# xingyizhou/CenterNet

Measured on AMD Instinct MI355X. Metric: images/sec whole-node, 512x512 ctdet, higher is better.
Workload: dtype f32s; 1 GPU; ctdet resdcn_18 512x512, batch 32 per GPU (BASELINE configs[1]), network + fused sigmoid/peak-NMS/top-K decode, K=100; global_batch=32, parallelism=image-sharded x1

## Files before the change

### centernet_amd/csrc/cn_proj.hip

```cpp
#include "cn_internal.h"
#include "cn_tuning.h"

namespace {

constexpr int J_NT = 256;
constexpr int J_NB = 4;
constexpr int J_ROW = 144;
constexpr int J_STRIP = 32 * J_ROW;
constexpr int J_SLOT = 32 * 128;
static_assert(J_STRIP <= 2 * J_SLOT, "the epilogue strip aliases the input slots");

struct JArgs {
    const char *x;
    const char *w;
    int ncb;
    const float *scale, *shift;
    char *y;
    int M, Ho, Wo, H, W, stride;
    int in_pitchB, out_pitchB, cout_pad, nchunk, Cout, relu;
    uint32_t *range;
};

typedef _Float16 j_f16x8 __attribute__((ext_vector_type(8)));

typedef __attribute__((address_space(3))) void j_lds_void;
typedef __attribute__((address_space(1))) const void j_glb_void;

template <bool OUT_PLAIN, int J_PRE>
__global__ __launch_bounds__(J_NT, 2) void proj1x1_kernel(const JArgs a)
{
    constexpr int J_WAVE = J_PRE * J_SLOT;
    constexpr int J_SS = 4 * J_WAVE;
    extern __shared__ __attribute__((aligned(128))) char smem[];
    const int tid = threadIdx.x, lane = tid & 63;
    const int wave = __builtin_amdgcn_readfirstlane(tid >> 6);
    const int l31 = lane & 31, h = lane >> 5;
    const int n0 = (int)blockIdx.y * (32 * J_NB);
    {
        const int which = tid >> 7, c = tid & 127;
        const float *src = which ? a.shift : a.scale;
        float v = which ? 0.f : 1.f;
        if (src && n0 + c < a.Cout) v = src[n0 + c];
        reinterpret_cast<float *>(smem + J_SS)[tid] = v;
    }
    const int m_base = (int)blockIdx.x * 128 + wave * 32;
    unsigned src_off[4];
#pragma unroll
    for (int q = 0; q < 4; ++q) {
        const int p = 8 * q + (lane >> 3);
        const int mc = min(m_base + p, a.M - 1);
        const int ox = mc % a.Wo, t1 = mc / a.Wo, oy = t1 % a.Ho, b = t1 / a.Ho;
        const unsigned pin = (unsigned)((b * a.H + oy * a.stride) * a.W + ox * a.stride);
        src_off[q] = pin * (unsigned)a.in_pitchB + (unsigned)(((lane & 7) ^ ((p >> 1) & 7)) * 16);
    }
    char *wbase = smem + wave * J_WAVE;
    auto dma = [&](int slot, int c) {
#pragma unroll
        for (int q = 0; q < 4; ++q)
            __builtin_amdgcn_global_load_lds((j_glb_void *)(a.x + src_off[q] + (unsigned)c * 128u),
                                             (j_lds_void *)(wbase + slot * J_SLOT + q * 1024), 16, 0, 0);
    };
#pragma unroll
    for (int c = 0; c < J_PRE; ++c)
        if (c < a.nchunk) dma(c, c);
    const int sw = (l31 >> 1) & 7;
    const int rd = l31 * 128;
    const char *wl = a.w + (size_t)(n0 >> 5) * 4096 + (unsigned)lane * 16u;
    const size_t chunkB = (size_t)a.ncb * 4096;
    const int nbv = min(J_NB, a.ncb - (n0 >> 5));

    cn_f32x16 acc[J_NB];
#pragma unroll
    for (int nb = 0; nb < J_NB; ++nb)
#pragma unroll
        for (int r = 0; r < 16; ++r) acc[nb][r] = 0.f;
    __syncthreads();

    for (int c = 0; c < a.nchunk; ++c) {
        const int slot = c & (J_PRE - 1);
        j_f16x8 af[2][4];
        auto load_a = [&](int set, int nb) {
            const char *g = wl + (size_t)c * chunkB + (size_t)min(nb, nbv - 1) * 4096;
#pragma unroll
            for (int qd = 0; qd < 4; ++qd) af[set][qd] = *reinterpret_cast<const j_f16x8 *>(g + qd * 1024);
        };
        load_a(0, 0);
        {
            const int younger = min(a.nchunk - 1 - c, J_PRE - 1);
            if (J_PRE > 2 && younger >= 3) asm volatile("s_waitcnt vmcnt(16)" ::: "memory");
            else if (J_PRE > 2 && younger == 2) asm volatile("s_waitcnt vmcnt(12)" ::: "memory");
            else if (younger == 1) asm volatile("s_waitcnt vmcnt(8)" ::: "memory");
            else asm volatile("s_waitcnt vmcnt(4)" ::: "memory");
        }
        j_f16x8 bf[4];
        {
            const char *sp = wbase + slot * J_SLOT + rd;
            bf[0] = *reinterpret_cast<const j_f16x8 *>(sp + (((0 + h) ^ sw) << 4));
            bf[1] = *reinterpret_cast<const j_f16x8 *>(sp + (((2 + h) ^ sw) << 4));
            bf[2] = *reinterpret_cast<const j_f16x8 *>(sp + (((4 + h) ^ sw) << 4));
            bf[3] = *reinterpret_cast<const j_f16x8 *>(sp + (((6 + h) ^ sw) << 4));
        }
#pragma unroll
        for (int nb = 0; nb < J_NB; ++nb) {
            const int set = nb & 1;
            if (nb + 1 < J_NB) load_a(set ^ 1, nb + 1);
            __builtin_amdgcn_sched_barrier(0);
#pragma unroll
            for (int kh = 0; kh < 2; ++kh) {
                acc[nb] = __builtin_amdgcn_mfma_f32_32x32x16_f16(af[set][2 + kh], bf[kh], acc[nb], 0, 0, 0);
                acc[nb] = __builtin_amdgcn_mfma_f32_32x32x16_f16(af[set][kh], bf[2 + kh], acc[nb], 0, 0, 0);
                acc[nb] = __builtin_amdgcn_mfma_f32_32x32x16_f16(af[set][kh], bf[kh], acc[nb], 0, 0, 0);
            }
            __builtin_amdgcn_sched_barrier(0);
        }
        if (c + J_PRE < a.nchunk) {
            asm volatile("s_waitcnt lgkmcnt(0)" ::: "memory");
            dma(slot, c + J_PRE);
        }
    }
    asm volatile("s_waitcnt vmcnt(0) lgkmcnt(0)" ::: "memory");

    char *strip = smem + wave * J_WAVE;
    const float *ss = reinterpret_cast<const float *>(smem + J_SS);
    float rng_out = 0.f;
    const int rrow = lane >> 3, rcol = lane & 7;
    const float floor_v = a.relu ? 0.f : -__builtin_inff();
#pragma unroll
    for (int nb = 0; nb < J_NB; ++nb) {
        if (n0 + 32 * nb >= a.cout_pad) break;
#pragma unroll
        for (int g = 0; g < 4; ++g) {
            const cn_f32x4 sc = *reinterpret_cast<const cn_f32x4 *>(ss + 32 * nb + 8 * g + 4 * h);
            const cn_f32x4 sh = *reinterpret_cast<const cn_f32x4 *>(ss + 128 + 32 * nb + 8 * g + 4 * h);
            cn_f32x4 v;
#pragma unroll
            for (int e = 0; e < 4; ++e) v[e] = fmaxf(acc[nb][4 * g + e] * sc[e] + sh[e], floor_v);
            if (OUT_PLAIN) {
                *reinterpret_cast<cn_f32x4 *>(strip + l31 * J_ROW + (8 * g + 4 * h) * 4) = v;
            } else {
                cn_rng_upd4(rng_out, v);
                cn_f16x4v h4, l4;
                cn_split4(v, h4, l4);
                *reinterpret_cast<cn_f16x4v *>(strip + l31 * J_ROW + (8 * g + 4 * h) * 2) = h4;
                *reinterpret_cast<cn_f16x4v *>(strip + l31 * J_ROW + 64 + (8 * g + 4 * h) * 2) = l4;
            }
        }
        asm volatile("" ::: "memory");
#pragma unroll
        for (int k = 0; k < 4; ++k) {
            const int row = 8 * k + rrow;
            const cn_f32x4 v = *reinterpret_cast<const cn_f32x4 *>(strip + row * J_ROW + rcol * 16);
            const int mo = (int)blockIdx.x * 128 + wave * 32 + row;
            if (mo < a.M)
                *reinterpret_cast<cn_f32x4 *>(a.y + (size_t)mo * a.out_pitchB + (size_t)(n0 + 32 * nb) * 4 + rcol * 16) = v;
        }
        asm volatile("" ::: "memory");
    }
    if (!OUT_PLAIN) cn_rng_commit(a.range, 0, rng_out);
}

}

bool cn_proj1x1_takes(const ConvCall &c)
{
    if (!cn_knobs.proj) return false;
    if ((c.Cin & 31) || (c.in_pitch & 31) || (c.out_pitch & 31) || (c.stride != 1 && c.stride != 2)) return false;
    if (c.out_pitch < c.cout_pad) return false;
    if ((size_t)c.B * c.H * c.W * c.in_pitch * 4 >= ((size_t)1 << 32)) return false;
    return c.Cin <= 1024 && c.Cout >= 32;
}

int cn_proj1x1_f32s(const ConvCall &c, hipStream_t st)
{
    JArgs a = {};
    a.x = (const char *)c.x; a.w = (const char *)c.w + (size_t)c.cout_pad * c.Cin * 4; a.scale = c.scale; a.shift = c.shift;
    a.y = (char *)c.y;
    a.H = c.H; a.W = c.W; a.stride = c.stride;
    a.Ho = c.Ho; a.Wo = c.Wo;
    a.M = c.B * a.Ho * a.Wo;
    a.in_pitchB = c.in_pitch * 4; a.out_pitchB = c.out_pitch * 4;
    a.cout_pad = c.cout_pad;
    a.ncb = a.cout_pad / 32;
    a.nchunk = c.Cin / 32;
    a.Cout = c.Cout; a.relu = c.relu;
    a.range = c.ctl ? c.ctl->range : nullptr;
    const dim3 grid((unsigned)cn_cdiv(a.M, 128), (unsigned)cn_cdiv(a.cout_pad, 32 * J_NB));
    const int pre = a.nchunk <= 2 ? 2 : 4;
    const int lds = 4 * pre * J_SLOT + 2 * 128 * 4;
    if (c.out_plain && pre == 2) {
        CN_SET_MAX_LDS_ONCE((proj1x1_kernel<true, 2>), 4 * 2 * J_SLOT + 1024);
        hipLaunchKernelGGL((proj1x1_kernel<true, 2>), grid, dim3(J_NT), lds, st, a);
    } else if (c.out_plain) {
        CN_SET_MAX_LDS_ONCE((proj1x1_kernel<true, 4>), 4 * 4 * J_SLOT + 1024);
        hipLaunchKernelGGL((proj1x1_kernel<true, 4>), grid, dim3(J_NT), lds, st, a);
    } else if (pre == 2) {
        CN_SET_MAX_LDS_ONCE((proj1x1_kernel<false, 2>), 4 * 2 * J_SLOT + 1024);
        hipLaunchKernelGGL((proj1x1_kernel<false, 2>), grid, dim3(J_NT), lds, st, a);
    } else {
        CN_SET_MAX_LDS_ONCE((proj1x1_kernel<false, 4>), 4 * 4 * J_SLOT + 1024);
        hipLaunchKernelGGL((proj1x1_kernel<false, 4>), grid, dim3(J_NT), lds, st, a);
    }
    CN_CHECK_LAUNCH();
    return CN_OK;
}
```

### centernet_amd/csrc/cn_tuning.h

```cpp
#pragma once

struct CnTuning {
    int nbuf, narrow, bm, nosplit, nostem, swz, setprio, dbgskip, nohalo, stem_persist, dcn_split, bm256, waves8,
        split_min_chunks, split_max, stagger_pct, occ4, f32s_lds_weights, f32s_policy, dcn_tile2d, dcn_form,
        heads_remap, heads_reg, stem16s, c3p, c3p_stagger, c3p_knobs, c3p_heads, c3p_deconv, c3p_s2, dcn_team,
        dcn_team_wgs, dcn_team_stagger, offconv, offconv_teams1, dcn_wide, dcn_wide_wgs, stem_dbg, stem_stagger,
        dcn_wide_prefetch, proj, c3p_grid, conv16h;
};
extern CnTuning cn_knobs;

struct CnTuningKey {
    int key;
    int CnTuning::*field;
    int def;
    int lo, hi;
    int n_also, also[4];
};

constexpr CnTuningKey CN_TUNING_KEYS[] = {
    {1, &CnTuning::nbuf, 0, 0, 2},
    {2, &CnTuning::narrow, 0, 0, 1},
    {3, nullptr, 0, 0, 0, 1, {64}},
    {4, &CnTuning::bm, 0, 0, 0, 2, {64, 128}},
    {5, &CnTuning::nosplit, 0, 0, 1},
    {6, &CnTuning::nostem, 0, 0, 1},
    {7, &CnTuning::swz, 0, 0, 2},
    {8, &CnTuning::setprio, 1, 0, 1},
    {9, &CnTuning::dbgskip, 0, 0, 2047},
    {10, &CnTuning::nohalo, 0, 0, 1},
    {11, nullptr, 0, 0, 0},
    {12, &CnTuning::stem_persist, 1, 0, 1},
    {13, &CnTuning::dcn_split, 0, 0, 1, 2, {3, 9}},
    {16, &CnTuning::split_min_chunks, 8, 1, 64},
    {17, &CnTuning::split_max, 16, 1, 64},
    {22, &CnTuning::dcn_tile2d, 1, 0, 1},
    {23, &CnTuning::dcn_form, 0, 0, 2, 4, {4, 5, 6, 7}},
    {27, &CnTuning::stem16s, 1, 0, 1},
    {14, &CnTuning::bm256, 0, 0, 3},
    {15, &CnTuning::waves8, 1, 0, 1},
    {18, &CnTuning::stagger_pct, 100, 0, 255},
    {19, &CnTuning::occ4, 0, 0, 2},
    {20, &CnTuning::f32s_lds_weights, 1, 0, 1},
    {21, &CnTuning::f32s_policy, 0, 0, 7},
    {24, &CnTuning::heads_remap, 1, 0, 3},
    {26, &CnTuning::heads_reg, 1, 0, 3},
    {28, &CnTuning::c3p, 1, 0, 7},
    {29, &CnTuning::c3p_stagger, 0, 0, 255},
    {30, &CnTuning::c3p_knobs, 2, 0, 255},
    {31, &CnTuning::c3p_heads, 1, 0, 1},
    {32, &CnTuning::c3p_deconv, 1, 0, 1},
    {33, &CnTuning::c3p_s2, 1, 0, 1},
    {47, &CnTuning::c3p_grid, 64, 1, 64},
    {36, &CnTuning::dcn_team, 3, 0, 3},
    {37, &CnTuning::dcn_team_wgs, 512, 1, 4096},
    {38, &CnTuning::dcn_team_stagger, 32, 0, 1024},
    {39, &CnTuning::offconv, 1, 0, 1},
    {40, &CnTuning::offconv_teams1, 768, 0, 1000000},
    {41, &CnTuning::dcn_wide, 1, 0, 1},
    {42, &CnTuning::dcn_wide_wgs, 256, 1, 4096},
    {45, &CnTuning::dcn_wide_prefetch, 1, 0, 1},
    {43, &CnTuning::stem_dbg, 0, 0, 31},
    {44, &CnTuning::stem_stagger, 0, 0, 1024},
    {46, &CnTuning::proj, 1, 0, 1},
    {65, &CnTuning::conv16h, 1, 0, 1},
};

constexpr CnTuning cn_tuning_defaults()
{
    CnTuning t = {};
    for (const CnTuningKey &k : CN_TUNING_KEYS)
        if (k.field) t.*k.field = k.def;
    return t;
}
```

Baseline: 13250 img/s.

## Split 1x1 projection into 8-wave blocks with wave pairs sharing input tiles

Rewrites the 1x1 projection conv kernel to use 512 threads, where each pair of waves shares one 32-row input strip in LDS and each wave covers two of the four 32-channel output blocks instead of all four. DMA loads of the input are split across the pair and synchronized with block barriers. Weight loads are software-pipelined across chunks. The aim is to halve per-wave accumulator and register pressure and spread the input staging over more waves to improve latency hiding. The cost is a barrier on every K chunk and a larger, reorganized LDS footprint. The old kernel stays available behind a new proj_form knob.

```diff
diff --git a/centernet_amd/csrc/cn_proj.hip b/centernet_amd/csrc/cn_proj.hip
--- a/centernet_amd/csrc/cn_proj.hip
+++ b/centernet_amd/csrc/cn_proj.hip
@@ -1,14 +1,19 @@
 #include "cn_internal.h"
 #include "cn_tuning.h"
+#include <type_traits>
 
 namespace {
 
-constexpr int J_NT = 256;
-constexpr int J_NB = 4;
+constexpr int J_NT = 512;
+constexpr int J_NB = 2;
+constexpr int J_WGN = 128;
+constexpr int JP_NT = 256;
+constexpr int JP_NB = 4;
 constexpr int J_ROW = 144;
 constexpr int J_STRIP = 32 * J_ROW;
 constexpr int J_SLOT = 32 * 128;
-static_assert(J_STRIP <= 2 * J_SLOT, "the epilogue strip aliases the input slots");
+constexpr int j_pair_bytes(int pre) { return pre * J_SLOT > 2 * J_STRIP ? pre * J_SLOT : 2 * J_STRIP; }
+static_assert(J_STRIP <= 2 * J_SLOT, "previous form: the epilogue strip aliases the wave's input slots");
 
 struct JArgs {
     const char *x;
@@ -26,9 +31,165 @@
 typedef __attribute__((address_space(3))) void j_lds_void;
 typedef __attribute__((address_space(1))) const void j_glb_void;
 
+__device__ __forceinline__ void j_barrier()
+{
+    asm volatile("" ::: "memory");
+    __builtin_amdgcn_s_barrier();
+    asm volatile("" ::: "memory");
+}
+
 template <bool OUT_PLAIN, int J_PRE>
 __global__ __launch_bounds__(J_NT, 2) void proj1x1_kernel(const JArgs a)
 {
+    constexpr int J_PAIR = j_pair_bytes(J_PRE);
+    constexpr int J_SS = 4 * J_PAIR;
+    extern __shared__ __attribute__((aligned(128))) char smem[];
+    const int tid = threadIdx.x, lane = tid & 63;
+    const int wave = __builtin_amdgcn_readfirstlane(tid >> 6);
+    const int pb = wave >> 1, ch = wave & 1;
+    const int l31 = lane & 31, h = lane >> 5;
+    const int n0 = (int)blockIdx.y * J_WGN;
+    const int nw = n0 + 32 * J_NB * ch;
+    if (tid < 2 * J_WGN) {
+        const int which = tid >> 7, c = tid & 127;
+        const float *src = which ? a.shift : a.scale;
+        float v = which ? 0.f : 1.f;
+        if (src && n0 + c < a.Cout) v = src[n0 + c];
+        reinterpret_cast<float *>(smem + J_SS)[tid] = v;
+    }
+    const int m_base = (int)blockIdx.x * 128 + pb * 32;
+    unsigned src_off[2];
+#pragma unroll
+    for (int j = 0; j < 2; ++j) {
+        const int p = 8 * (2 * ch + j) + (lane >> 3);
+        const int mc = min(m_base + p, a.M - 1);
+        const int ox = mc % a.Wo, t1 = mc / a.Wo, oy = t1 % a.Ho, b = t1 / a.Ho;
+        const unsigned pin = (unsigned)((b * a.H + oy * a.stride) * a.W + ox * a.stride);
+        src_off[j] = pin * (unsigned)a.in_pitchB + (unsigned)(((lane & 7) ^ ((p >> 1) & 7)) * 16);
+    }
+    char *pbase = smem + pb * J_PAIR;
+    auto dma = [&](int slot, int c) {
+#pragma unroll
+        for (int j = 0; j < 2; ++j)
+            __builtin_amdgcn_global_load_lds((j_glb_void *)(a.x + src_off[j] + (unsigned)c * 128u),
+                                             (j_lds_void *)(pbase + slot * J_SLOT + (2 * ch + j) * 1024), 16, 0, 0);
+    };
+    const int sw = (l31 >> 1) & 7;
+    const int rd = l31 * 128;
+    const char *wl = a.w + (unsigned)lane * 16u;
+    const size_t chunkB = (size_t)a.ncb * 4096;
+    unsigned boff[J_NB];
+#pragma unroll
+    for (int nb = 0; nb < J_NB; ++nb) boff[nb] = (unsigned)min((nw >> 5) + nb, a.ncb - 1) * 4096u;
+    j_f16x8 af[J_NB][4];
+    auto load_a = [&](int nb, int c) {
+        const char *g = wl + (size_t)c * chunkB + boff[nb];
+#pragma unroll
+        for (int qd = 0; qd < 4; ++qd) af[nb][qd] = *reinterpret_cast<const j_f16x8 *>(g + qd * 1024);
+    };
+
+    cn_f32x16 acc[J_NB];
+#pragma unroll
+    for (int nb = 0; nb < J_NB; ++nb)
+#pragma unroll
+        for (int r = 0; r < 16; ++r) acc[nb][r] = 0.f;
+
+    load_a(0, 0);
+    __builtin_amdgcn_sched_barrier(0);
+    const int npre = min(J_PRE, a.nchunk);
+#pragma unroll
+    for (int c = 0; c < J_PRE; ++c)
+        if (c < npre) dma(c, c);
+
+    auto mfma_block = [&](int nb, const j_f16x8 (&bf)[4]) {
+#pragma unroll
+        for (int kh = 0; kh < 2; ++kh) {
+            acc[nb] = __builtin_amdgcn_mfma_f32_32x32x16_f16(af[nb][2 + kh], bf[kh], acc[nb], 0, 0, 0);
+            acc[nb] = __builtin_amdgcn_mfma_f32_32x32x16_f16(af[nb][kh], bf[2 + kh], acc[nb], 0, 0, 0);
+            acc[nb] = __builtin_amdgcn_mfma_f32_32x32x16_f16(af[nb][kh], bf[kh], acc[nb], 0, 0, 0);
+        }
+    };
+    auto chunk = [&](int c, auto refill) {
+        const int slot = c & (J_PRE - 1);
+        if (c == 0) {
+            if (npre >= 4) asm volatile("s_waitcnt vmcnt(6)" ::: "memory");
+            else if (npre == 3) asm volatile("s_waitcnt vmcnt(4)" ::: "memory");
+            else if (npre == 2) asm volatile("s_waitcnt vmcnt(2)" ::: "memory");
+            else asm volatile("s_waitcnt vmcnt(0)" ::: "memory");
+        } else {
+            asm volatile("s_waitcnt vmcnt(4)" ::: "memory");
+        }
+        asm volatile("s_waitcnt lgkmcnt(0)" ::: "memory");
+        j_barrier();
+        load_a(1, c);
+        if (decltype(refill)::value) dma((c - 1) & (J_PRE - 1), c - 1 + J_PRE);
+        j_f16x8 bf[4];
+        {
+            const char *sp = pbase + slot * J_SLOT + rd;
+            bf[0] = *reinterpret_cast<const j_f16x8 *>(sp + (((0 + h) ^ sw) << 4));
+            bf[1] = *reinterpret_cast<const j_f16x8 *>(sp + (((2 + h) ^ sw) << 4));
+            bf[2] = *reinterpret_cast<const j_f16x8 *>(sp + (((4 + h) ^ sw) << 4));
+            bf[3] = *reinterpret_cast<const j_f16x8 *>(sp + (((6 + h) ^ sw) << 4));
+        }
+        __builtin_amdgcn_sched_barrier(0);
+        mfma_block(0, bf);
+        __builtin_amdgcn_sched_barrier(0);
+        load_a(0, min(c + 1, a.nchunk - 1));
+        __builtin_amdgcn_sched_barrier(0);
+        mfma_block(1, bf);
+        __builtin_amdgcn_sched_barrier(0);
+    };
+    chunk(0, std::false_type{});
+    int c = 1;
+    if constexpr (J_PRE > 2)
+        for (; c <= a.nchunk - J_PRE; ++c) chunk(c, std::true_type{});
+    for (; c < a.nchunk; ++c) chunk(c, std::false_type{});
+    asm volatile("s_waitcnt vmcnt(0) lgkmcnt(0)" ::: "memory");
+    j_barrier();
+
+    char *strip = pbase + ch * J_STRIP;
+    const float *ss = reinterpret_cast<const float *>(smem + J_SS) + 32 * J_NB * ch;
+    float rng_out = 0.f;
+    const int rrow = lane >> 3, rcol = lane & 7;
+    const float floor_v = a.relu ? 0.f : -__builtin_inff();
+#pragma unroll
+    for (int nb = 0; nb < J_NB; ++nb) {
+        if (nw + 32 * nb >= a.cout_pad) break;
+#pragma unroll
+        for (int g = 0; g < 4; ++g) {
+            const cn_f32x4 sc = *reinterpret_cast<const cn_f32x4 *>(ss + 32 * nb + 8 * g + 4 * h);
+            const cn_f32x4 sh = *reinterpret_cast<const cn_f32x4 *>(ss + J_WGN + 32 * nb + 8 * g + 4 * h);
+            cn_f32x4 v;
+#pragma unroll
+            for (int e = 0; e < 4; ++e) v[e] = fmaxf(acc[nb][4 * g + e] * sc[e] + sh[e], floor_v);
+            if (OUT_PLAIN) {
+                *reinterpret_cast<cn_f32x4 *>(strip + l31 * J_ROW + (8 * g + 4 * h) * 4) = v;
+            } else {
+                cn_rng_upd4(rng_out, v);
+                cn_f16x4v h4, l4;
+                cn_split4(v, h4, l4);
+                *reinterpret_cast<cn_f16x4v *>(strip + l31 * J_ROW + (8 * g + 4 * h) * 2) = h4;
+                *reinterpret_cast<cn_f16x4v *>(strip + l31 * J_ROW + 64 + (8 * g + 4 * h) * 2) = l4;
+            }
+        }
+        asm volatile("" ::: "memory");
+#pragma unroll
+        for (int k = 0; k < 4; ++k) {
+            const int row = 8 * k + rrow;
+            const cn_f32x4 v = *reinterpret_cast<const cn_f32x4 *>(strip + row * J_ROW + rcol * 16);
+            const int mo = m_base + row;
+            if (mo < a.M)
+                *reinterpret_cast<cn_f32x4 *>(a.y + (size_t)mo * a.out_pitchB + (size_t)(nw + 32 * nb) * 4 + rcol * 16) = v;
+        }
+        asm volatile("" ::: "memory");
+    }
+    if (!OUT_PLAIN) cn_rng_commit(a.range, 0, rng_out);
+}
+
+template <bool OUT_PLAIN, int J_PRE>
+__global__ __launch_bounds__(JP_NT, 2) void proj1x1_prev_kernel(const JArgs a)
+{
+    constexpr int J_NB = JP_NB;
     constexpr int J_WAVE = J_PRE * J_SLOT;
     constexpr int J_SS = 4 * J_WAVE;
     extern __shared__ __attribute__((aligned(128))) char smem[];
@@ -184,22 +345,26 @@
     a.nchunk = c.Cin / 32;
     a.Cout = c.Cout; a.relu = c.relu;
     a.range = c.ctl ? c.ctl->range : nullptr;
-    const dim3 grid((unsigned)cn_cdiv(a.M, 128), (unsigned)cn_cdiv(a.cout_pad, 32 * J_NB));
+    const dim3 grid((unsigned)cn_cdiv(a.M, 128), (unsigned)cn_cdiv(a.cout_pad, J_WGN));
     const int pre = a.nchunk <= 2 ? 2 : 4;
-    const int lds = 4 * pre * J_SLOT + 2 * 128 * 4;
-    if (c.out_plain && pre == 2) {
-        CN_SET_MAX_LDS_ONCE((proj1x1_kernel<true, 2>), 4 * 2 * J_SLOT + 1024);
-        hipLaunchKernelGGL((proj1x1_kernel<true, 2>), grid, dim3(J_NT), lds, st, a);
-    } else if (c.out_plain) {
-        CN_SET_MAX_LDS_ONCE((proj1x1_kernel<true, 4>), 4 * 4 * J_SLOT + 1024);
-        hipLaunchKernelGGL((proj1x1_kernel<true, 4>), grid, dim3(J_NT), lds, st, a);
-    } else if (pre == 2) {
-        CN_SET_MAX_LDS_ONCE((proj1x1_kernel<false, 2>), 4 * 2 * J_SLOT + 1024);
-        hipLaunchKernelGGL((proj1x1_kernel<false, 2>), grid, dim3(J_NT), lds, st, a);
-    } else {
-        CN_SET_MAX_LDS_ONCE((proj1x1_kernel<false, 4>), 4 * 4 * J_SLOT + 1024);
-        hipLaunchKernelGGL((proj1x1_kernel<false, 4>), grid, dim3(J_NT), lds, st, a);
-    }
+#define J_LAUNCH(KERNEL, NT, PLAIN, PRE, BYTES)                                                  \
+    do {                                                                                         \
+        CN_SET_MAX_LDS_ONCE((KERNEL<PLAIN, PRE>), (BYTES));                                      \
+        hipLaunchKernelGGL((KERNEL<PLAIN, PRE>), grid, dim3(NT), (BYTES), st, a);                \
+    } while (0)
+#define J_LAUNCH_FORM(KERNEL, NT, BYTES2, BYTES4)                                                \
+    do {                                                                                         \
+        if (c.out_plain && pre == 2) J_LAUNCH(KERNEL, NT, true, 2, BYTES2);                      \
+        else if (c.out_plain) J_LAUNCH(KERNEL, NT, true, 4, BYTES4);                             \
+        else if (pre == 2) J_LAUNCH(KERNEL, NT, false, 2, BYTES2);                               \
+        else J_LAUNCH(KERNEL, NT, false, 4, BYTES4);                                             \
+    } while (0)
+    if (cn_knobs.proj_form == 1)
+        J_LAUNCH_FORM(proj1x1_prev_kernel, JP_NT, 4 * 2 * J_SLOT + 1024, 4 * 4 * J_SLOT + 1024);
+    else
+        J_LAUNCH_FORM(proj1x1_kernel, J_NT, 4 * j_pair_bytes(2) + 1024, 4 * j_pair_bytes(4) + 1024);
+#undef J_LAUNCH_FORM
+#undef J_LAUNCH
     CN_CHECK_LAUNCH();
     return CN_OK;
 }
diff --git a/centernet_amd/csrc/cn_tuning.h b/centernet_amd/csrc/cn_tuning.h
--- a/centernet_amd/csrc/cn_tuning.h
+++ b/centernet_amd/csrc/cn_tuning.h
@@ -5,7 +5,7 @@
         split_min_chunks, split_max, stagger_pct, occ4, f32s_lds_weights, f32s_policy, dcn_tile2d, dcn_form,
         heads_remap, heads_reg, stem16s, c3p, c3p_stagger, c3p_knobs, c3p_heads, c3p_deconv, c3p_s2, dcn_team,
         dcn_team_wgs, dcn_team_stagger, offconv, offconv_teams1, dcn_wide, dcn_wide_wgs, stem_dbg, stem_stagger,
-        dcn_wide_prefetch, proj, c3p_grid, conv16h;
+        dcn_wide_prefetch, proj, c3p_grid, conv16h, proj_form;
 };
 extern CnTuning cn_knobs;
 
@@ -63,6 +63,7 @@
     {44, &CnTuning::stem_stagger, 0, 0, 1024},
     {46, &CnTuning::proj, 1, 0, 1},
     {65, &CnTuning::conv16h, 1, 0, 1},
+    {66, &CnTuning::proj_form, 0, 0, 1},
 };
 
 constexpr CnTuning cn_tuning_defaults()
```

Measured after the change: 13220 img/s. No clear change (-0.3%).
